# bbc/turingcodec

Measured on AMD Instinct MI355X. Metric: encoded fps (havoc hot path, primitive-batch throughput: one picture's primitive calls per frame as whole-frame batches;, higher is better.
Workload: dtype u8; 1 GPU; 1920x1080 8-bit 4:2:0 random-access QP32 speed=medium B-frame, MEASURED call mix of the reference encoder on this clip generator (profiles/r04_reference_call_mi; calls_per_frame=3944815, launches_per_frame=49, pictures_in_flight=2, parallelism=single GPU

## Files before the change

### turingcodec_amd/csrc/kernels_tu_fused.hip

```cpp
#include "common.h"

#include <cstdlib>
#include "transform_basis.h"
#include "launch.h"
#include "rdoq_work.h"

namespace havoc_gpu {

template <int S, int N>
__device__ __forceinline__ void load_sample_row(const char *p, uint32_t (&row)[N / 2])
{
    if (S == 1)
    {
        uint32_t b[N / 4];
        if (N == 4) b[0] = ld4(p);
        else if (N == 8)
        {
            const u32x2 v = ld8(p);
            b[0] = v.x; b[1] = v.y;
        }
        else
        {
#pragma unroll
            for (int q = 0; q < N / 16; ++q)
            {
                const u32x4 v = ld16(p + 16 * q);
                b[4 * q] = v.x; b[4 * q + 1] = v.y; b[4 * q + 2] = v.z; b[4 * q + 3] = v.w;
            }
        }
#pragma unroll
        for (int q = 0; q < N / 4; ++q)
        {
            row[2 * q] = __builtin_amdgcn_perm(0u, b[q], 0x0c010c00u);
            row[2 * q + 1] = __builtin_amdgcn_perm(0u, b[q], 0x0c030c02u);
        }
    }
    else
    {
        if (N == 4)
        {
            const u32x2 v = ld8(p);
            row[0] = v.x; row[1] = v.y;
        }
        else
        {
#pragma unroll
            for (int q = 0; q < N / 8; ++q)
            {
                const u32x4 v = ld16(p + 16 * q);
                row[4 * q] = v.x; row[4 * q + 1] = v.y; row[4 * q + 2] = v.z; row[4 * q + 3] = v.w;
            }
        }
    }
}

template <int S, int LOG2, int TR, bool SCAN = false>
__global__ __launch_bounds__(64) void k_tu_forward(int16_t *__restrict__ coeffs, const char *__restrict__ src, long stride_src,
                                                   const char *__restrict__ pred, long stride_pred, const int32_t *__restrict__ jobs, int njobs,
                                                   int bitDepth, const RdoqJob *__restrict__ rjobs = nullptr, int16_t *__restrict__ levels = nullptr,
                                                   RdoqWork *__restrict__ work = nullptr)
{
    constexpr int N = 1 << LOG2, TPW = 64 / N, LS = N + 2;
    __shared__ int16_t lds[TPW][N * LS];
    const int t = threadIdx.x / N, r = threadIdx.x % N;
    const int job = xcd_block(blockIdx.x, gridDim.x) * TPW + t;
    const bool live = job < njobs;
    const int32_t *j = jobs + (long)(live ? job : 0) * 4;
    const int shift1 = LOG2 - 1 + bitDepth - 8, shift2 = LOG2 + 6;

    uint32_t row[N / 2], prow[N / 2];
    load_sample_row<S, N>(src + ((long)j[1] + (long)r * stride_src) * S, row);
    load_sample_row<S, N>(pred + ((long)j[2] + (long)r * stride_pred) * S, prow);
#pragma unroll
    for (int p = 0; p < N / 2; ++p) row[p] = pk_sub(row[p], prow[p]);
    int o[N];
    basis_times_row<N, TR, false, true>(row, 1 << (shift1 - 1), o);
#pragma unroll
    for (int k = 0; k < N; ++k) lds[t][k * LS + r] = (int16_t)(o[k] >> shift1);
    __syncthreads();
#pragma unroll
    for (int p = 0; p < N / 2; ++p) row[p] = *reinterpret_cast<const uint32_t *>(&lds[t][r * LS + 2 * p]);
    basis_times_row<N, TR, false>(row, 1 << (shift2 - 1), o);
    if (SCAN)
    {
        constexpr int GW = N / 4;
        const RdoqJob rj = rjobs[live ? job : 0];
        uint32_t thr[3];
        rdoqThresholds(rj.quant_scale, rj.quant_shift, thr);
        uint32_t lo = 0, hi = 0;
        uint64_t mask[3] = {0, 0, 0};
#pragma unroll
        for (int gy = 0; gy < GW; ++gy)
        {
            uint32_t big = 0;
#pragma unroll
            for (int k = 4 * gy; k < 4 * gy + 4; ++k)
            {
                const int c = (int16_t)(o[k] >> shift2);
                big = max(big, (uint32_t)abs(c));
                const uint32_t sq = (uint32_t)(c * c);
                lo += sq & 0xffffu;
                hi += sq >> 16;
            }
            big = max(big, (uint32_t)__shfl_xor((int)big, 1, kWave));
            big = max(big, (uint32_t)__shfl_xor((int)big, 2, kWave));
#pragma unroll
            for (int m = 0; m < 3; ++m)
            {
                const uint64_t b = __ballot(live && (r & 3) == 0 && big >= thr[m]) >> (t * N);
                uint32_t f = 0;
#pragma unroll
                for (int gx = 0; gx < GW; ++gx) f |= (uint32_t)((b >> (4 * gx)) & 1) << gx;
                mask[m] |= (uint64_t)f << (gy * GW);
            }
        }
        const int slo = group_sum<N>((int)lo), shi = group_sum<N>((int)hi);
        if (live)
        {
            int16_t *z = levels + rj.dst_off + r * N;
#pragma unroll
            for (int q = 0; q < N / 4; ++q) st8(z + 4 * q, u32x2{0, 0});
            if (r == 0)
            {
                RdoqInfo *info = reinterpret_cast<RdoqInfo *>(reinterpret_cast<char *>(work) + rdoqInfoOffset());
                RdoqInfo v;
                v.mask = mask[0];
                v.mask2 = mask[1];
                v.mask3 = mask[2];
                v.sumSq = ((int64_t)shi << 16) + slo;
                info[job] = v;
            }
        }
    }
    if (!live) return;
    int16_t *c = coeffs + j[0] + r;
#pragma unroll
    for (int k = 0; k < N; ++k) c[k * N] = (int16_t)(o[k] >> shift2);
}

template <int S, int LOG2, int TR>
__global__ __launch_bounds__(64) void k_tu_reconstruct(char *rec, long stride_rec, const char *pred, long stride_pred, const char *__restrict__ src,
                                                       long stride_src, const int16_t *__restrict__ levels, const int32_t *__restrict__ jobs,
                                                       int njobs, int bitDepth, int scale, int shift, uint32_t *__restrict__ ssd)
{
    typedef typename Sample<S>::T T;
    constexpr int N = 1 << LOG2, TPW = 64 / N, LS = N + 2;
    __shared__ int16_t lds[TPW][N * LS];
    const int t = threadIdx.x / N, r = threadIdx.x % N;
    const int job = xcd_block(blockIdx.x, gridDim.x) * TPW + t;
    const bool live = job < njobs;
    const int32_t *j = jobs + (long)(live ? job : 0) * 4;
    const int shift2 = 20 - bitDepth;
    const int dqadd = 1 << (shift - 1);

    const int16_t *c = levels + j[0] + r;
    uint32_t col[N / 2];
#pragma unroll
    for (int p = 0; p < N / 2; ++p)
    {
        const int lo = clip3(-32768, 32767, ((int)c[(2 * p) * N] * scale + dqadd) >> shift);
        const int hi = clip3(-32768, 32767, ((int)c[(2 * p + 1) * N] * scale + dqadd) >> shift);
        col[p] = ((uint32_t)lo & 0xffffu) | ((uint32_t)hi << 16);
    }
    int o[N];
    basis_times_row<N, TR, true>(col, 1 << 6, o);
#pragma unroll
    for (int k = 0; k < N; ++k) lds[t][k * LS + r] = (int16_t)clip3(-32768, 32767, o[k] >> 7);
    __syncthreads();
#pragma unroll
    for (int p = 0; p < N / 2; ++p) col[p] = *reinterpret_cast<const uint32_t *>(&lds[t][r * LS + 2 * p]);
    basis_times_row<N, TR, true>(col, 1 << (shift2 - 1), o);

    const int maxv = (1 << bitDepth) - 1;
    uint32_t prow[N / 2], srow[N / 2];
    load_sample_row<S, N>(pred + ((long)j[2] + (long)r * stride_pred) * S, prow);
    load_sample_row<S, N>(src + ((long)j[1] + (long)r * stride_src) * S, srow);
    uint32_t acc = 0;
    int v[N];
#pragma unroll
    for (int k = 0; k < N; ++k)
    {
        const int res = clip3(-32768, 32767, o[k] >> shift2);
        const int pk = (k & 1) ? (int)(prow[k >> 1] >> 16) : (int)(prow[k >> 1] & 0xffff);
        const int sk = (k & 1) ? (int)(srow[k >> 1] >> 16) : (int)(srow[k >> 1] & 0xffff);
        v[k] = clip3(0, maxv, pk + res);
        const int d = sk - v[k];
        acc += (uint32_t)(d * d);
    }
    if (live)
    {
        T *q = reinterpret_cast<T *>(rec) + j[3] + (long)r * stride_rec;
        if (S == 1)
        {
#pragma unroll
            for (int k = 0; k < N; k += 4) st4(q + k, (uint32_t)v[k] | ((uint32_t)v[k + 1] << 8) | ((uint32_t)v[k + 2] << 16) | ((uint32_t)v[k + 3] << 24));
        }
        else
        {
#pragma unroll
            for (int k = 0; k < N; k += 2) st4(q + k, (uint32_t)v[k] | ((uint32_t)v[k + 1] << 16));
        }
    }
    uint32_t tot = (uint32_t)group_sum<N>((int)acc);
    if (S == 2) tot >>= 4;
    if (live && r == 0) ssd[job] = tot;
}

template <int S, int LOG2>
__global__ __launch_bounds__(64) void k_intra_measure(int16_t *__restrict__ coeffs, int16_t *__restrict__ coeffsDct, int32_t *__restrict__ satd, char *__restrict__ rec0,
                                                      uint32_t *__restrict__ ssd0, const char *__restrict__ src, long stride_src, const char *__restrict__ pred,
                                                      long stride_pred, const int32_t *__restrict__ jobs, int njobs, int bitDepth, int withSatd)
{
    typedef typename Sample<S>::T T;
    constexpr int N = 1 << LOG2, TPW = 64 / N, LS = N + 2, TS = N >= 8 ? 8 : 4, TX = N / TS, TILES = TX * TX;
    __shared__ int16_t lds[TPW][N * LS];
    const int t = threadIdx.x / N, r = threadIdx.x % N;
    const int job = blockIdx.x * TPW + t;
    const bool live = job < njobs;
    const int32_t *j = jobs + (long)(live ? job : 0) * 4;
    const int shift1 = LOG2 - 1 + bitDepth - 8, shift2 = LOG2 + 6;

    uint32_t row[N / 2], prow[N / 2];
    load_sample_row<S, N>(src + ((long)j[1] + (long)r * stride_src) * S, row);
    load_sample_row<S, N>(pred + ((long)j[2] + (long)r * stride_pred) * S, prow);
    if (live)
    {
        const int maxv = (1 << bitDepth) - 1;
        T *q = reinterpret_cast<T *>(rec0) + j[3] + (long)r * N;
#pragma unroll
        for (int p = 0; p < N / 2; ++p)
        {
            q[2 * p] = (T)clip3(0, maxv, (int)(prow[p] & 0xffff));
            q[2 * p + 1] = (T)clip3(0, maxv, (int)(prow[p] >> 16));
        }
    }
#pragma unroll
    for (int p = 0; p < N / 2; ++p) row[p] = pk_sub(row[p], prow[p]);
    {
        uint32_t acc = 0;
#pragma unroll
        for (int p = 0; p < N / 2; ++p)
        {
            const int lo = (int16_t)(row[p] & 0xffff), hi = (int16_t)(row[p] >> 16);
            acc += (uint32_t)(lo * lo) + (uint32_t)(hi * hi);
        }
        uint32_t tot = (uint32_t)group_sum<N>((int)acc);
        if (S == 2) tot >>= 4;
        if (live && r == 0) ssd0[job] = tot;
    }
    if (withSatd)
    {
#pragma unroll
        for (int tx = 0; tx < TX; ++tx)
        {
            int c;
            if (S == 1)
            {
                uint32_t p[TS / 2];
#pragma unroll
                for (int k = 0; k < TS / 2; ++k) p[k] = row[tx * (TS / 2) + k];
                c = satd_rows_pk<TS>(p, r & (TS - 1));
            }
            else
            {
                int d[TS];
#pragma unroll
                for (int k = 0; k < TS / 2; ++k)
                {
                    d[2 * k] = (int16_t)(row[tx * (TS / 2) + k] & 0xffff);
                    d[2 * k + 1] = (int16_t)(row[tx * (TS / 2) + k] >> 16);
                }
                c = satd_rows<S, TS>(d, r & (TS - 1));
            }
            if (live && (r & (TS - 1)) == 0) satd[(long)job * TILES + (r / TS) * TX + tx] = c;
        }
    }
    uint32_t keep[N / 2];
#pragma unroll
    for (int p = 0; p < N / 2; ++p) keep[p] = row[p];
    int o[N];
    constexpr int TR = LOG2 == 2 ? 1 : 0;
    basis_times_row<N, TR, false, true>(row, 1 << (shift1 - 1), o);
#pragma unroll
    for (int k = 0; k < N; ++k) lds[t][k * LS + r] = (int16_t)(o[k] >> shift1);
    __syncthreads();
#pragma unroll
    for (int p = 0; p < N / 2; ++p) row[p] = *reinterpret_cast<const uint32_t *>(&lds[t][r * LS + 2 * p]);
    basis_times_row<N, TR, false>(row, 1 << (shift2 - 1), o);
    if (live)
    {
        int16_t *c = coeffs + j[0] + r;
#pragma unroll
        for (int k = 0; k < N; ++k) c[k * N] = (int16_t)(o[k] >> shift2);
    }
    if (LOG2 == 2)
    {
        __syncthreads();
        basis_times_row<N, 0, false, true>(keep, 1 << (shift1 - 1), o);
#pragma unroll
        for (int k = 0; k < N; ++k) lds[t][k * LS + r] = (int16_t)(o[k] >> shift1);
        __syncthreads();
#pragma unroll
        for (int p = 0; p < N / 2; ++p) row[p] = *reinterpret_cast<const uint32_t *>(&lds[t][r * LS + 2 * p]);
        basis_times_row<N, 0, false>(row, 1 << (shift2 - 1), o);
        if (live)
        {
            int16_t *c = coeffsDct + j[0] + r;
#pragma unroll
            for (int k = 0; k < N; ++k) c[k * N] = (int16_t)(o[k] >> shift2);
        }
    }
}

hipError_t launch_intra_measure(hipStream_t st, int S, int bd, int log2, int16_t *coeffs, int16_t *coeffsDct, int32_t *satd, void *rec0, uint32_t *ssd0, const void *src,
                                long ss, const void *pred, long sp, const havoc_mi355x_tu_fused_job *jobs, int n, int withSatd)
{
    if (n <= 0) return hipSuccess;
    if (log2 < 2 || log2 > 5) return hipErrorInvalidValue;
    const int tpw = 64 >> log2;
    const dim3 g((n + tpw - 1) / tpw), b(64);
    char *r0 = (char *)rec0;
    const char *s8 = (const char *)src, *p8 = (const char *)pred;
    const int32_t *j = (const int32_t *)jobs;
#define MEASURE_GO(SS, LL) hipLaunchKernelGGL((k_intra_measure<SS, LL>), g, b, 0, st, coeffs, coeffsDct, satd, r0, ssd0, s8, ss, p8, sp, j, n, bd, withSatd)
    if (S == 1) { if (log2 == 2) MEASURE_GO(1, 2); else if (log2 == 3) MEASURE_GO(1, 3); else if (log2 == 4) MEASURE_GO(1, 4); else MEASURE_GO(1, 5); }
    else { if (log2 == 2) MEASURE_GO(2, 2); else if (log2 == 3) MEASURE_GO(2, 3); else if (log2 == 4) MEASURE_GO(2, 4); else MEASURE_GO(2, 5); }
#undef MEASURE_GO
    return hipGetLastError();
}


typedef int i32x16v __attribute__((ext_vector_type(16)));
typedef int i32x4v __attribute__((ext_vector_type(4)));

struct Dct32I8 { int8_t m[32][32]; int32_t rowsum128[32]; };
constexpr Dct32I8 make_dct32_i8()
{
    Dct32I8 t{};
    for (int k = 0; k < 32; ++k)
    {
        int sum = 0;
        for (int c = 0; c < 32; ++c)
        {
            t.m[k][c] = (int8_t)basis(32, 0, k, c);
            sum += basis(32, 0, k, c);
        }
        t.rowsum128[k] = 128 * sum;
    }
    return t;
}
static __constant__ Dct32I8 c_dct32_i8 = make_dct32_i8();

__device__ __forceinline__ void mfma_dct32(const i32x4v a, const uint32_t (&v)[8], int add, int half, int (&out)[16])
{
    i32x4v bh, bl;
#pragma unroll
    for (int q = 0; q < 4; ++q)
    {
        bh[q] = (int)__builtin_amdgcn_perm(v[2 * q + 1], v[2 * q], 0x07050301u);
        bl[q] = (int)(__builtin_amdgcn_perm(v[2 * q + 1], v[2 * q], 0x06040200u) ^ 0x80808080u);
    }
    i32x16v ch, cl;
#pragma unroll
    for (int reg = 0; reg < 16; ++reg)
    {
        ch[reg] = 0;
        cl[reg] = add + c_dct32_i8.rowsum128[(reg & 3) + 8 * (reg >> 2) + 4 * half];
    }
    ch = __builtin_amdgcn_mfma_i32_32x32x32_i8(a, bh, ch, 0, 0, 0);
    cl = __builtin_amdgcn_mfma_i32_32x32x32_i8(a, bl, cl, 0, 0, 0);
#pragma unroll
    for (int reg = 0; reg < 16; ++reg) out[reg] = (int)(((uint32_t)ch[reg] << 8) + (uint32_t)cl[reg]);
}

template <bool SCAN>
__global__ __launch_bounds__(64) void k_tu_forward_mfma32(int16_t *__restrict__ coeffs, const char *__restrict__ src, long stride_src, const char *__restrict__ pred,
                                                          long stride_pred, const int32_t *__restrict__ jobs, int njobs, const RdoqJob *__restrict__ rjobs = nullptr,
                                                          int16_t *__restrict__ levels = nullptr, RdoqWork *__restrict__ work = nullptr)
{
    constexpr int LS = 40;
    __shared__ __attribute__((aligned(16))) int16_t lds[32 * LS];
    const int job = xcd_block(blockIdx.x, gridDim.x);
    if (job >= njobs) return;
    const int32_t *j = jobs + (long)job * 4;
    const int lane = threadIdx.x, y = lane & 31, half = lane >> 5;
    const i32x4v a = *reinterpret_cast<const i32x4v *>(&c_dct32_i8.m[y][16 * half]);
    uint32_t r[8];
    {
        const u32x4 s4 = ld16(src + (long)j[1] + (long)y * stride_src + 16 * half), p4 = ld16(pred + (long)j[2] + (long)y * stride_pred + 16 * half);
        const uint32_t sw[4] = {s4.x, s4.y, s4.z, s4.w}, pw[4] = {p4.x, p4.y, p4.z, p4.w};
#pragma unroll
        for (int q = 0; q < 4; ++q)
        {
            r[2 * q] = pk_sub(__builtin_amdgcn_perm(0u, sw[q], 0x0c010c00u), __builtin_amdgcn_perm(0u, pw[q], 0x0c010c00u));
            r[2 * q + 1] = pk_sub(__builtin_amdgcn_perm(0u, sw[q], 0x0c030c02u), __builtin_amdgcn_perm(0u, pw[q], 0x0c030c02u));
        }
    }
    int t[16];
    mfma_dct32(a, r, 8, half, t);
#pragma unroll
    for (int reg = 0; reg < 16; ++reg) lds[((reg & 3) + 8 * (reg >> 2) + 4 * half) * LS + y] = (int16_t)(t[reg] >> 4);
    __syncthreads();
    uint32_t v[8];
    {
        const u32x4 q0 = *reinterpret_cast<const u32x4 *>(&lds[y * LS + 16 * half]), q1 = *reinterpret_cast<const u32x4 *>(&lds[y * LS + 16 * half + 8]);
        v[0] = q0.x; v[1] = q0.y; v[2] = q0.z; v[3] = q0.w; v[4] = q1.x; v[5] = q1.y; v[6] = q1.z; v[7] = q1.w;
    }
    int o[16];
    mfma_dct32(a, v, 1024, half, o);
    int16_t *c = coeffs + j[0] + y;
#pragma unroll
    for (int reg = 0; reg < 16; ++reg) c[((reg & 3) + 8 * (reg >> 2) + 4 * half) * 32] = (int16_t)(o[reg] >> 11);
    if (SCAN)
    {
        const RdoqJob rj = rjobs[job];
        uint32_t thr[3];
        rdoqThresholds(rj.quant_scale, rj.quant_shift, thr);
        uint32_t lo = 0, hi = 0;
        uint64_t mask[3] = {0, 0, 0};
#pragma unroll
        for (int q = 0; q < 4; ++q)
        {
            uint32_t big = 0;
#pragma unroll
            for (int k = 0; k < 4; ++k)
            {
                const int cf = (int16_t)(o[4 * q + k] >> 11);
                big = max(big, (uint32_t)abs(cf));
                const uint32_t sq = (uint32_t)(cf * cf);
                lo += sq & 0xffffu;
                hi += sq >> 16;
            }
            big = max(big, (uint32_t)__shfl_xor((int)big, 1, kWave));
            big = max(big, (uint32_t)__shfl_xor((int)big, 2, kWave));
#pragma unroll
            for (int m = 0; m < 3; ++m)
            {
                const uint64_t b = __ballot((y & 3) == 0 && big >= thr[m]);
                uint32_t f0 = 0, f1 = 0;
#pragma unroll
                for (int gx = 0; gx < 8; ++gx)
                {
                    f0 |= (uint32_t)((b >> (4 * gx)) & 1) << gx;
                    f1 |= (uint32_t)((b >> (32 + 4 * gx)) & 1) << gx;
                }
                mask[m] |= (uint64_t)f0 << (16 * q) | (uint64_t)f1 << (16 * q + 8);
            }
        }
        const int slo = wave_sum((int)lo), shi = wave_sum((int)hi);
        int16_t *z = levels + rj.dst_off + lane * 16;
        st8(z, u32x2{0, 0}); st8(z + 4, u32x2{0, 0}); st8(z + 8, u32x2{0, 0}); st8(z + 12, u32x2{0, 0});
        if (lane == 0)
        {
            RdoqInfo *info = reinterpret_cast<RdoqInfo *>(reinterpret_cast<char *>(work) + rdoqInfoOffset());
            RdoqInfo w;
            w.mask = mask[0];
            w.mask2 = mask[1];
            w.mask3 = mask[2];
            w.sumSq = ((int64_t)shi << 16) + slo;
            info[job] = w;
        }
    }
}

static bool mfmaForward()
{
    static const bool on = !(getenv("HAVOC_TU_MFMA") && atoi(getenv("HAVOC_TU_MFMA")) == 0);
    return on;
}

template <int S, int LOG2, int TR>
static void go_fwd(hipStream_t st, int16_t *co, const char *src, long ss, const char *pred, long sp, const int32_t *j, int n, int bd)
{
    constexpr int TPW = 64 >> LOG2;
    hipLaunchKernelGGL((k_tu_forward<S, LOG2, TR>), dim3((n + TPW - 1) / TPW), dim3(64), 0, st, co, src, ss, pred, sp, j, n, bd);
}

template <int S>
static hipError_t launch_fwd_s(hipStream_t st, int bd, int log2, int tr, int16_t *co, const char *src, long ss, const char *pred, long sp,
                               const int32_t *j, int n)
{
    if (tr)
    {
        if (log2 != 2) return hipErrorInvalidValue;
        go_fwd<S, 2, 1>(st, co, src, ss, pred, sp, j, n, bd);
    }
    else
        switch (log2)
        {
        case 2: go_fwd<S, 2, 0>(st, co, src, ss, pred, sp, j, n, bd); break;
        case 3: go_fwd<S, 3, 0>(st, co, src, ss, pred, sp, j, n, bd); break;
        case 4: go_fwd<S, 4, 0>(st, co, src, ss, pred, sp, j, n, bd); break;
        case 5:
            if (S == 1 && bd == 8 && mfmaForward()) hipLaunchKernelGGL((k_tu_forward_mfma32<false>), dim3(n), dim3(64), 0, st, co, src, ss, pred, sp, j, n);
            else go_fwd<S, 5, 0>(st, co, src, ss, pred, sp, j, n, bd);
            break;
        default: return hipErrorInvalidValue;
        }
    return hipGetLastError();
}

hipError_t launch_tu_forward_scan(hipStream_t st, int S, int bd, int log2, int16_t *coeffs, const void *src, long ss, const void *pred, long sp,
                                  const havoc_mi355x_tu_fused_job *jobs, int n, const RdoqJob *rj, int16_t *levels, void *workspace)
{
    if (n <= 0) return hipSuccess;
    if (log2 != 4 && log2 != 5) return hipErrorInvalidValue;
    const char *s8 = (const char *)src, *p8 = (const char *)pred;
    const int32_t *j = (const int32_t *)jobs;
    RdoqWork *w = (RdoqWork *)workspace;
    const int tpw = 64 >> log2;
    const dim3 g((n + tpw - 1) / tpw), b(64);
    if (S == 1 && log2 == 4) hipLaunchKernelGGL((k_tu_forward<1, 4, 0, true>), g, b, 0, st, coeffs, s8, ss, p8, sp, j, n, bd, rj, levels, w);
    else if (S == 1 && bd == 8 && mfmaForward()) hipLaunchKernelGGL((k_tu_forward_mfma32<true>), dim3(n), b, 0, st, coeffs, s8, ss, p8, sp, j, n, rj, levels, w);
    else if (S == 1) hipLaunchKernelGGL((k_tu_forward<1, 5, 0, true>), g, b, 0, st, coeffs, s8, ss, p8, sp, j, n, bd, rj, levels, w);
    else if (log2 == 4) hipLaunchKernelGGL((k_tu_forward<2, 4, 0, true>), g, b, 0, st, coeffs, s8, ss, p8, sp, j, n, bd, rj, levels, w);
    else hipLaunchKernelGGL((k_tu_forward<2, 5, 0, true>), g, b, 0, st, coeffs, s8, ss, p8, sp, j, n, bd, rj, levels, w);
    return hipGetLastError();
}

hipError_t launch_tu_forward(hipStream_t st, int S, int bd, int log2, int tr, int16_t *coeffs, const void *src, long ss, const void *pred, long sp,
                             const havoc_mi355x_tu_fused_job *jobs, int n)
{
    if (n <= 0) return hipSuccess;
    return S == 1 ? launch_fwd_s<1>(st, bd, log2, tr, coeffs, (const char *)src, ss, (const char *)pred, sp, (const int32_t *)jobs, n)
                  : launch_fwd_s<2>(st, bd, log2, tr, coeffs, (const char *)src, ss, (const char *)pred, sp, (const int32_t *)jobs, n);
}

template <int S, int LOG2, int TR>
static void go_rec(hipStream_t st, char *rec, long sr, const char *pred, long sp, const char *src, long ss, const int16_t *lv, const int32_t *j, int n,
                   int bd, int scale, int shift, uint32_t *ssd)
{
    constexpr int TPW = 64 >> LOG2;
    hipLaunchKernelGGL((k_tu_reconstruct<S, LOG2, TR>), dim3((n + TPW - 1) / TPW), dim3(64), 0, st, rec, sr, pred, sp, src, ss, lv, j, n, bd, scale,
                       shift, ssd);
}

template <int S>
static hipError_t launch_rec_s(hipStream_t st, int bd, int log2, int tr, int scale, int shift, char *rec, long sr, const char *pred, long sp,
                               const char *src, long ss, const int16_t *lv, const int32_t *j, int n, uint32_t *ssd)
{
    if (tr)
    {
        if (log2 != 2) return hipErrorInvalidValue;
        go_rec<S, 2, 1>(st, rec, sr, pred, sp, src, ss, lv, j, n, bd, scale, shift, ssd);
    }
    else
        switch (log2)
        {
        case 2: go_rec<S, 2, 0>(st, rec, sr, pred, sp, src, ss, lv, j, n, bd, scale, shift, ssd); break;
        case 3: go_rec<S, 3, 0>(st, rec, sr, pred, sp, src, ss, lv, j, n, bd, scale, shift, ssd); break;
        case 4: go_rec<S, 4, 0>(st, rec, sr, pred, sp, src, ss, lv, j, n, bd, scale, shift, ssd); break;
        case 5: go_rec<S, 5, 0>(st, rec, sr, pred, sp, src, ss, lv, j, n, bd, scale, shift, ssd); break;
        default: return hipErrorInvalidValue;
        }
    return hipGetLastError();
}

hipError_t launch_tu_reconstruct(hipStream_t st, int S, int bd, int log2, int tr, int scale, int shift, void *rec, long sr, const void *pred, long sp,
                                 const void *src, long ss, const int16_t *levels, const havoc_mi355x_tu_fused_job *jobs, int n, uint32_t *ssd)
{
    if (n <= 0) return hipSuccess;
    return S == 1 ? launch_rec_s<1>(st, bd, log2, tr, scale, shift, (char *)rec, sr, (const char *)pred, sp, (const char *)src, ss, levels,
                                    (const int32_t *)jobs, n, ssd)
                  : launch_rec_s<2>(st, bd, log2, tr, scale, shift, (char *)rec, sr, (const char *)pred, sp, (const char *)src, ss, levels,
                                    (const int32_t *)jobs, n, ssd);
}

}
```

### turingcodec_amd/csrc/transform_basis.h

```cpp
#pragma once

#include "common.h"

namespace havoc_gpu {

constexpr int kMag[33] = {64, 90, 90, 90, 89, 88, 87, 85, 83, 82, 80, 78, 75, 73, 70, 67, 64,
                          61, 57, 54, 50, 46, 43, 38, 36, 31, 25, 22, 18, 13, 9,  4,  0};
constexpr int kDst7[4][4] = {{29, 55, 74, 84}, {74, 74, 0, -74}, {84, -29, -74, 55}, {55, -84, 74, -29}};

constexpr int basis(int n, int tr, int k, int c)
{
    if (tr) return kDst7[k][c];
    const int kk = k * (32 / n);
    if (kk == 0) return 64;
    const int j = (kk * (2 * c + 1)) & 127;
    return j <= 32 ? kMag[j] : (j <= 64 ? -kMag[64 - j] : (j <= 96 ? -kMag[j - 64] : kMag[128 - j]));
}

template <int N> struct PackedBasis { uint32_t v[N][N / 2]; };

template <int N, int TR, bool INV>
constexpr PackedBasis<N> make_basis()
{
    PackedBasis<N> m{};
    for (int k = 0; k < N; ++k)
        for (int p = 0; p < N / 2; ++p)
        {
            const int lo = INV ? basis(N, TR, 2 * p, k) : basis(N, TR, k, 2 * p);
            const int hi = INV ? basis(N, TR, 2 * p + 1, k) : basis(N, TR, k, 2 * p + 1);
            m.v[k][p] = ((uint32_t)lo & 0xffffu) | ((uint32_t)hi << 16);
        }
    return m;
}

static __constant__ PackedBasis<4> c_fwd_dst4 = make_basis<4, 1, false>();
static __constant__ PackedBasis<4> c_fwd_dct4 = make_basis<4, 0, false>();
static __constant__ PackedBasis<8> c_fwd_dct8 = make_basis<8, 0, false>();
static __constant__ PackedBasis<16> c_fwd_dct16 = make_basis<16, 0, false>();
static __constant__ PackedBasis<32> c_fwd_dct32 = make_basis<32, 0, false>();
static __constant__ PackedBasis<4> c_inv_dst4 = make_basis<4, 1, true>();
static __constant__ PackedBasis<4> c_inv_dct4 = make_basis<4, 0, true>();
static __constant__ PackedBasis<8> c_inv_dct8 = make_basis<8, 0, true>();
static __constant__ PackedBasis<16> c_inv_dct16 = make_basis<16, 0, true>();
static __constant__ PackedBasis<32> c_inv_dct32 = make_basis<32, 0, true>();

template <int N, int TR, bool INV> __device__ __forceinline__ const PackedBasis<N> &basis_table();
template <> __device__ __forceinline__ const PackedBasis<4> &basis_table<4, 1, false>() { return c_fwd_dst4; }
template <> __device__ __forceinline__ const PackedBasis<4> &basis_table<4, 0, false>() { return c_fwd_dct4; }
template <> __device__ __forceinline__ const PackedBasis<8> &basis_table<8, 0, false>() { return c_fwd_dct8; }
template <> __device__ __forceinline__ const PackedBasis<16> &basis_table<16, 0, false>() { return c_fwd_dct16; }
template <> __device__ __forceinline__ const PackedBasis<32> &basis_table<32, 0, false>() { return c_fwd_dct32; }
template <> __device__ __forceinline__ const PackedBasis<4> &basis_table<4, 1, true>() { return c_inv_dst4; }
template <> __device__ __forceinline__ const PackedBasis<4> &basis_table<4, 0, true>() { return c_inv_dct4; }
template <> __device__ __forceinline__ const PackedBasis<8> &basis_table<8, 0, true>() { return c_inv_dct8; }
template <> __device__ __forceinline__ const PackedBasis<16> &basis_table<16, 0, true>() { return c_inv_dct16; }
template <> __device__ __forceinline__ const PackedBasis<32> &basis_table<32, 0, true>() { return c_inv_dct32; }

__device__ __forceinline__ int dot2(uint32_t a, uint32_t b, int c)
{
    return __builtin_amdgcn_sdot2(__builtin_bit_cast(s16x2, a), __builtin_bit_cast(s16x2, b), c, false);
}


template <int N> struct PackedBasisEO { uint32_t ve[N / 2][N / 4], vo[N / 2][N / 4]; };

template <int N>
constexpr PackedBasisEO<N> make_basis_eo()
{
    PackedBasisEO<N> m{};
    for (int i = 0; i < N / 2; ++i)
        for (int q = 0; q < N / 4; ++q)
        {
            m.ve[i][q] = ((uint32_t)basis(N, 0, 4 * q, i) & 0xffffu) | ((uint32_t)basis(N, 0, 4 * q + 2, i) << 16);
            m.vo[i][q] = ((uint32_t)basis(N, 0, 4 * q + 1, i) & 0xffffu) | ((uint32_t)basis(N, 0, 4 * q + 3, i) << 16);
        }
    return m;
}
static __constant__ PackedBasisEO<16> c_eo_dct16 = make_basis_eo<16>();
static __constant__ PackedBasisEO<32> c_eo_dct32 = make_basis_eo<32>();
template <int N> __device__ __forceinline__ const PackedBasisEO<N> &basis_eo();
template <> __device__ __forceinline__ const PackedBasisEO<16> &basis_eo<16>() { return c_eo_dct16; }
template <> __device__ __forceinline__ const PackedBasisEO<32> &basis_eo<32>() { return c_eo_dct32; }

template <int N, int TR, bool INV, bool FOLD = false>
__device__ __forceinline__ void basis_times_row(const uint32_t (&row)[N / 2], int add, int (&out)[N])
{
    if constexpr (INV && TR == 0 && N >= 16)
    {
        const PackedBasisEO<N> &m = basis_eo<N>();
        uint32_t ce[N / 4], co[N / 4];
#pragma unroll
        for (int q = 0; q < N / 4; ++q)
        {
            ce[q] = __builtin_amdgcn_perm(row[2 * q + 1], row[2 * q], 0x05040100u);
            co[q] = __builtin_amdgcn_perm(row[2 * q + 1], row[2 * q], 0x07060302u);
        }
#pragma unroll
        for (int i = 0; i < N / 2; ++i)
        {
            int e = add, o = 0;
#pragma unroll
            for (int q = 0; q < N / 4; ++q)
            {
                e = dot2(ce[q], m.ve[i][q], e);
                o = dot2(co[q], m.vo[i][q], o);
            }
            out[i] = e + o;
            out[N - 1 - i] = e - o;
        }
    }
    else if constexpr (!INV && TR == 0 && N >= 16 && FOLD)
    {
        const PackedBasis<N> &m = basis_table<N, TR, INV>();
        uint32_t ev[N / 4], od[N / 4];
#pragma unroll
        for (int p = 0; p < N / 4; ++p)
        {
            const uint32_t b = row[N / 2 - 1 - p];
            const uint32_t bs = __builtin_amdgcn_alignbit(b, b, 16);
            ev[p] = pk_add(row[p], bs);
            od[p] = pk_sub(row[p], bs);
        }
#pragma unroll
        for (int k = 0; k < N; ++k)
        {
            int a = add;
#pragma unroll
            for (int p = 0; p < N / 4; ++p) a = dot2((k & 1) ? od[p] : ev[p], m.v[k][p], a);
            out[k] = a;
        }
    }
    else
    {
        const PackedBasis<N> &m = basis_table<N, TR, INV>();
#pragma unroll
        for (int k = 0; k < N; ++k)
        {
            int a = add;
#pragma unroll
            for (int p = 0; p < N / 2; ++p) a = dot2(row[p], m.v[k][p], a);
            out[k] = a;
        }
    }
}

template <int N>
__device__ __forceinline__ void load_row16(const int16_t *p, uint32_t (&row)[N / 2])
{
    if (N == 4)
    {
        const u32x2 v = ld8(p);
        row[0] = v.x; row[1] = v.y;
    }
    else
    {
#pragma unroll
        for (int q = 0; q < N / 8; ++q)
        {
            const u32x4 v = ld16(p + 8 * q);
            row[4 * q] = v.x; row[4 * q + 1] = v.y; row[4 * q + 2] = v.z; row[4 * q + 3] = v.w;
        }
    }
}

}
```

Before: 1610 frames/s.

## Skip zero coefficient regions in TU reconstruct via wavefront-uniform extent

The reconstruct kernel now finds, across the wavefront, the highest nonzero row and column band of the quantized levels using ballots. It dispatches truncated inverse-transform passes that only multiply over the first 4/8/16 inputs, and skips both passes when every level is zero. It also packs the add/clip/SSD math into 16-bit pairs with saturating ops and dot2, issues the pred/src loads early for small sizes, and reduces the SSD with DPP into the last lane. The cost is more template instantiations and branches, which means higher code size and register pressure. The savings depend on how sparse the levels are per wavefront.

```diff
diff --git a/profiles/level_extent.py b/profiles/level_extent.py
--- /dev/null
+++ b/profiles/level_extent.py
@@ -0,0 +1,72 @@
+#!/usr/bin/env python3
+import argparse
+import os
+import sys
+from collections import Counter
+
+import numpy as np
+
+ROOT = os.path.dirname(os.path.dirname(os.path.abspath(__file__)))
+sys.path.insert(0, ROOT)
+sys.path.insert(0, os.path.join(ROOT, "tests"))
+from turingcodec_amd.workload import FrameWorkload, quant_params, dequant_params
+from reflibs import Oracle
+
+
+def cls(k, n):
+    return 0 if k == 0 else next(c for c in (4, 8, 16, 32) if k <= c or c >= n)
+
+
+def levels_of(o, wl, g, log2, tr, i):
+    n, st = g["n"], wl.stride
+    so, po = int(g["src"][i, 0]), int(g["src"][i, 1])
+    sblk = np.stack([wl.luma[so + r * st: so + r * st + n] for r in range(n)]).astype(np.int32)
+    pblk = np.stack([wl.luma[po + r * st: po + r * st + n] for r in range(n)]).astype(np.int32)
+    res = np.ascontiguousarray((sblk - pblk).astype(np.int16).ravel())
+    coef = np.zeros(n * n, np.int16)
+    o.transform(coef, 0, res, 0, n, log2, tr, wl.bit_depth)
+    qs, qsh, _ = quant_params(wl.qp, log2, wl.bit_depth, False)
+    inv, _ = dequant_params(wl.qp, log2, wl.bit_depth)
+    lv, _ = o.rdoq(coef, log2, 0, int(g["scan_idx"][i]), int(g["is_intra"][i]), 1, qs, qsh, inv, wl.bit_depth, wl.rdoq_lambda, wl.rdoq_states[g["ctx_index"][i]])
+    return np.asarray(lv).reshape(n, n)
+
+
+def extents(wl, waves, seed=1):
+    o = Oracle()
+    rng = np.random.default_rng(seed)
+    out = {}
+    for (log2, tr), g in sorted(wl.tu.items()):
+        n = g["n"]
+        tpw = 64 // n
+        nw = len(g["jobs"]) // tpw
+        per_block, per_wave = Counter(), Counter()
+        for w in rng.choice(nw, min(waves, nw), replace=False):
+            kr = kc = 0
+            for i in range(w * tpw, (w + 1) * tpw):
+                nz = levels_of(o, wl, g, log2, tr, i) != 0
+                rows, cols = np.flatnonzero(nz.any(1)), np.flatnonzero(nz.any(0))
+                r, c = (cls(rows[-1] + 1, n), cls(cols[-1] + 1, n)) if len(rows) else (0, 0)
+                per_block[(r, c)] += 1
+                kr, kc = max(kr, r), max(kc, c)
+            per_wave[(kr, kc)] += 1
+        out[(log2, tr)] = (tpw, per_block, per_wave)
+    return out
+
+
+def show(c):
+    tot = sum(c.values())
+    return "  ".join(f"{'zero' if k == (0, 0) else '%dx%d' % k} {100.0 * v / tot:.1f}%" for k, v in sorted(c.items()))
+
+
+if __name__ == "__main__":
+    ap = argparse.ArgumentParser()
+    ap.add_argument("--qp", type=int, default=32)
+    ap.add_argument("--waves", type=int, default=300)
+    a = ap.parse_args()
+    wl = FrameWorkload(1920, 1080, 8, 11, qp=a.qp)
+    print(f"FrameWorkload(1920, 1080, 8, 11, qp={a.qp}): extent of the levels, rows x columns rounded up to 0 / 4 / 8 / 16 / N; {a.waves} wavefronts per size")
+    for (log2, tr), (tpw, blocks, waves) in extents(wl, a.waves).items():
+        n = 1 << log2
+        print(f"{n}x{n} {'DST' if tr else 'DCT'}  ({tpw} blocks per wavefront, {sum(blocks.values())} blocks sampled)")
+        print(f"    per block      {show(blocks)}")
+        print(f"    per wavefront  {show(waves)}")
diff --git a/profiles/r07/tu_reconstruct_sparse_counts.py b/profiles/r07/tu_reconstruct_sparse_counts.py
--- /dev/null
+++ b/profiles/r07/tu_reconstruct_sparse_counts.py
@@ -0,0 +1,42 @@
+#!/usr/bin/env python3
+import csv
+import glob
+import os
+import re
+import sys
+
+
+def rows(d, pattern):
+    for f in sorted(glob.glob(os.path.join(d, "**", pattern), recursive=True)):
+        with open(f) as fh:
+            yield from csv.DictReader(fh)
+
+
+def inst(name):
+    m = re.search(r"k_tu_reconstruct<([^>]*)>", name)
+    return m.group(1).replace(" ", "") if m else name
+
+
+def main(pmc, trace, steps):
+    launches = []
+    for r in rows(pmc, "*counter_collection.csv"):
+        if r.get("Counter_Name") == "SQ_INSTS_VALU" and "k_tu_reconstruct" in r["Kernel_Name"]:
+            launches.append((int(r.get("Dispatch_Id", len(launches))), inst(r["Kernel_Name"]), int(r.get("Grid_Size", 0)) // max(int(r.get("Workgroup_Size", 64)), 1),
+                             float(r["Counter_Value"])))
+    launches.sort()
+    per = len(launches) // steps if steps else len(launches)
+    print(f"{len(launches)} k_tu_reconstruct launches in {steps} steps ({per} per step); S, LOG2, TR | workgroups (one wavefront each) | SQ_INSTS_VALU | per wavefront")
+    for i, (_, k, wg, v) in enumerate(launches):
+        if steps and i % per == 0:
+            print(f"  step {i // per}")
+        print(f"    <{k}>  {wg:7d}  {v:12.0f}  {v / wg if wg else 0:8.1f}")
+    if launches:
+        print(f"  sum per step: {sum(v for *_, v in launches) / max(steps, 1):.0f}")
+    for r in rows(trace, "*kernel_stats.csv"):
+        if "k_tu_reconstruct" in r.get("Name", ""):
+            print(f"  trace <{inst(r['Name'])}>  calls {r.get('Calls')}  total {float(r.get('TotalDurationNs', 0)) / 1e3:.1f} us  average {float(r.get('AverageNs', 0)) / 1e3:.2f} us"
+                  f"  min {float(r.get('MinNs', 0)) / 1e3:.2f}  max {float(r.get('MaxNs', 0)) / 1e3:.2f}")
+
+
+if __name__ == "__main__":
+    main(sys.argv[1], sys.argv[2], int(sys.argv[3]) if len(sys.argv) > 3 else 2)
diff --git a/turingcodec_amd/csrc/kernels_tu_fused.hip b/turingcodec_amd/csrc/kernels_tu_fused.hip
--- a/turingcodec_amd/csrc/kernels_tu_fused.hip
+++ b/turingcodec_amd/csrc/kernels_tu_fused.hip
@@ -8,50 +8,47 @@
 namespace havoc_gpu {
 
 template <int S, int N>
-__device__ __forceinline__ void load_sample_row(const char *p, uint32_t (&row)[N / 2])
-{
-    if (S == 1)
-    {
-        uint32_t b[N / 4];
-        if (N == 4) b[0] = ld4(p);
-        else if (N == 8)
-        {
-            const u32x2 v = ld8(p);
-            b[0] = v.x; b[1] = v.y;
-        }
-        else
-        {
-#pragma unroll
-            for (int q = 0; q < N / 16; ++q)
-            {
-                const u32x4 v = ld16(p + 16 * q);
-                b[4 * q] = v.x; b[4 * q + 1] = v.y; b[4 * q + 2] = v.z; b[4 * q + 3] = v.w;
-            }
-        }
-#pragma unroll
-        for (int q = 0; q < N / 4; ++q)
+__device__ __forceinline__ void load_sample_bytes(const char *p, uint32_t (&b)[N * S / 4])
+{
+    constexpr int BYTES = N * S;
+    if (BYTES == 4) b[0] = ld4(p);
+    else if (BYTES == 8)
+    {
+        const u32x2 v = ld8(p);
+        b[0] = v.x; b[1] = v.y;
+    }
+    else
+    {
+#pragma unroll
+        for (int q = 0; q < BYTES / 16; ++q)
+        {
+            const u32x4 v = ld16(p + 16 * q);
+            b[4 * q] = v.x; b[4 * q + 1] = v.y; b[4 * q + 2] = v.z; b[4 * q + 3] = v.w;
+        }
+    }
+}
+
+template <int S, int N>
+__device__ __forceinline__ void unpack_sample_row(const uint32_t (&b)[N * S / 4], uint32_t (&row)[N / 2])
+{
+#pragma unroll
+    for (int q = 0; q < N * S / 4; ++q)
+    {
+        if (S == 1)
         {
             row[2 * q] = __builtin_amdgcn_perm(0u, b[q], 0x0c010c00u);
             row[2 * q + 1] = __builtin_amdgcn_perm(0u, b[q], 0x0c030c02u);
         }
-    }
-    else
-    {
-        if (N == 4)
-        {
-            const u32x2 v = ld8(p);
-            row[0] = v.x; row[1] = v.y;
-        }
-        else
-        {
-#pragma unroll
-            for (int q = 0; q < N / 8; ++q)
-            {
-                const u32x4 v = ld16(p + 16 * q);
-                row[4 * q] = v.x; row[4 * q + 1] = v.y; row[4 * q + 2] = v.z; row[4 * q + 3] = v.w;
-            }
-        }
-    }
+        else row[q] = b[q];
+    }
+}
+
+template <int S, int N>
+__device__ __forceinline__ void load_sample_row(const char *p, uint32_t (&row)[N / 2])
+{
+    uint32_t b[N * S / 4];
+    load_sample_bytes<S, N>(p, b);
+    unpack_sample_row<S, N>(b, row);
 }
 
 template <int S, int LOG2, int TR, bool SCAN = false>
@@ -138,6 +135,49 @@
     for (int k = 0; k < N; ++k) c[k * N] = (int16_t)(o[k] >> shift2);
 }
 
+template <int G>
+__device__ __forceinline__ int group_sum_last(int v)
+{
+    v += __builtin_amdgcn_update_dpp(0, v, 0x111, 0xf, 0xf, true);
+    v += __builtin_amdgcn_update_dpp(0, v, 0x112, 0xf, 0xf, true);
+    if (G >= 8) v += __builtin_amdgcn_update_dpp(0, v, 0x114, 0xf, 0xe, true);
+    if (G >= 16) v += __builtin_amdgcn_update_dpp(0, v, 0x118, 0xf, 0xc, true);
+    if (G >= 32) v += __builtin_amdgcn_update_dpp(0, v, 0x142, 0xa, 0xf, true);
+    return v;
+}
+
+__device__ __forceinline__ uint32_t pack_sat(int lo, int hi) { return __builtin_bit_cast(uint32_t, __builtin_amdgcn_cvt_pk_i16(lo, hi)); }
+
+template <int N, int TR, int KR>
+__device__ __forceinline__ void rec_pass1(const int (&lv)[N], int scale, int dqadd, int shift, int16_t *ldsCol)
+{
+    constexpr int LS = N + 2;
+    uint32_t col[N / 2];
+#pragma unroll
+    for (int p = 0; p < KR / 2; ++p) col[p] = pack_sat((lv[2 * p] * scale + dqadd) >> shift, (lv[2 * p + 1] * scale + dqadd) >> shift);
+    int o[N];
+    basis_times_row<N, TR, true, false, KR>(col, 1 << 6, o);
+#pragma unroll
+    for (int k = 0; k < N; k += 2)
+    {
+        const s16x2 pr = __builtin_amdgcn_cvt_pk_i16(o[k] >> 7, o[k + 1] >> 7);
+        ldsCol[k * LS] = pr.x;
+        ldsCol[(k + 1) * LS] = pr.y;
+    }
+}
+
+template <int N, int TR, int KC>
+__device__ __forceinline__ void rec_pass2(const int16_t *ldsRow, int shift2, uint32_t (&res)[N / 2])
+{
+    uint32_t row[N / 2];
+#pragma unroll
+    for (int p = 0; p < KC / 2; ++p) row[p] = *reinterpret_cast<const uint32_t *>(&ldsRow[2 * p]);
+    int o[N];
+    basis_times_row<N, TR, true, false, KC>(row, 1 << (shift2 - 1), o);
+#pragma unroll
+    for (int p = 0; p < N / 2; ++p) res[p] = pack_sat(o[2 * p] >> shift2, o[2 * p + 1] >> shift2);
+}
+
 template <int S, int LOG2, int TR>
 __global__ __launch_bounds__(64) void k_tu_reconstruct(char *rec, long stride_rec, const char *pred, long stride_pred, const char *__restrict__ src,
                                                        long stride_src, const int16_t *__restrict__ levels, const int32_t *__restrict__ jobs,
@@ -145,65 +185,109 @@
 {
     typedef typename Sample<S>::T T;
     constexpr int N = 1 << LOG2, TPW = 64 / N, LS = N + 2;
+    constexpr int K4 = 4, K8 = N < 8 ? N : 8, K16 = N < 16 ? N : 16;
     __shared__ int16_t lds[TPW][N * LS];
     const int t = threadIdx.x / N, r = threadIdx.x % N;
     const int job = xcd_block(blockIdx.x, gridDim.x) * TPW + t;
     const bool live = job < njobs;
     const int32_t *j = jobs + (long)(live ? job : 0) * 4;
+    const int coef_off = j[0], src_off = j[1], pred_off = j[2], rec_off = j[3];
     const int shift2 = 20 - bitDepth;
     const int dqadd = 1 << (shift - 1);
 
-    const int16_t *c = levels + j[0] + r;
-    uint32_t col[N / 2];
+    const int16_t *c = levels + coef_off + r;
+    int lv[N];
+#pragma unroll
+    for (int k = 0; k < N; ++k) lv[k] = c[k * N];
+    constexpr bool EARLY = N < 32;
+    const char *prow_at = pred + ((long)pred_off + (long)r * stride_pred) * S, *srow_at = src + ((long)src_off + (long)r * stride_src) * S;
+    uint32_t pbytes[N * S / 4], sbytes[N * S / 4];
+    if (EARLY)
+    {
+        load_sample_bytes<S, N>(prow_at, pbytes);
+        load_sample_bytes<S, N>(srow_at, sbytes);
+    }
+
+    int from16 = 0, from8 = 0, from4 = 0, any = 0;
+#pragma unroll
+    for (int k = 0; k < N; ++k)
+    {
+        if (k >= 16) from16 |= lv[k];
+        else if (k >= 8) from8 |= lv[k];
+        else if (k >= 4) from4 |= lv[k];
+        else any |= lv[k];
+    }
+    from8 |= from16;
+    from4 |= from8;
+    any |= from4;
+    const uint64_t lives = __builtin_amdgcn_ballot_w64(live);
+    uint64_t cols = __builtin_amdgcn_ballot_w64(any != 0) & lives;
+    const bool rows4 = (__builtin_amdgcn_ballot_w64(from4 != 0) & lives) != 0, rows8 = (__builtin_amdgcn_ballot_w64(from8 != 0) & lives) != 0,
+               rows16 = (__builtin_amdgcn_ballot_w64(from16 != 0) & lives) != 0;
+    const int kr = __builtin_amdgcn_readfirstlane(cols == 0 ? 0 : rows16 ? 32 : rows8 ? 16 : rows4 ? 8 : 4);
+#pragma unroll
+    for (int w = 32; w >= N; w >>= 1) cols |= cols >> w;
+    const uint32_t field = (uint32_t)cols & (uint32_t)((1ull << N) - 1);
+    const int kc = __builtin_amdgcn_readfirstlane(field == 0 ? 0 : (field >> 16) ? 32 : (field >> 8) ? 16 : (field >> 4) ? 8 : 4);
+
+    uint32_t res[N / 2];
+    if (kr == 0)
+    {
+#pragma unroll
+        for (int p = 0; p < N / 2; ++p) res[p] = 0;
+    }
+    else
+    {
+        int16_t *ldsCol = &lds[t][r];
+        if (kr <= K4) rec_pass1<N, TR, K4>(lv, scale, dqadd, shift, ldsCol);
+        else if (kr <= K8) rec_pass1<N, TR, K8>(lv, scale, dqadd, shift, ldsCol);
+        else if (kr <= K16) rec_pass1<N, TR, K16>(lv, scale, dqadd, shift, ldsCol);
+        else rec_pass1<N, TR, N>(lv, scale, dqadd, shift, ldsCol);
+        __syncthreads();
+        const int16_t *ldsRow = &lds[t][r * LS];
+        if (kc <= K4) rec_pass2<N, TR, K4>(ldsRow, shift2, res);
+        else if (kc <= K8) rec_pass2<N, TR, K8>(ldsRow, shift2, res);
+        else if (kc <= K16) rec_pass2<N, TR, K16>(ldsRow, shift2, res);
+        else rec_pass2<N, TR, N>(ldsRow, shift2, res);
+    }
+
+    const uint32_t maxv = (uint32_t)((1 << bitDepth) - 1) * 0x10001u;
+    if (!EARLY)
+    {
+        load_sample_bytes<S, N>(prow_at, pbytes);
+        load_sample_bytes<S, N>(srow_at, sbytes);
+    }
+    uint32_t prow[N / 2], srow[N / 2];
+    unpack_sample_row<S, N>(pbytes, prow);
+    unpack_sample_row<S, N>(sbytes, srow);
+    int acc = 0;
+    uint32_t v[N / 2];
 #pragma unroll
     for (int p = 0; p < N / 2; ++p)
     {
-        const int lo = clip3(-32768, 32767, ((int)c[(2 * p) * N] * scale + dqadd) >> shift);
-        const int hi = clip3(-32768, 32767, ((int)c[(2 * p + 1) * N] * scale + dqadd) >> shift);
-        col[p] = ((uint32_t)lo & 0xffffu) | ((uint32_t)hi << 16);
-    }
-    int o[N];
-    basis_times_row<N, TR, true>(col, 1 << 6, o);
-#pragma unroll
-    for (int k = 0; k < N; ++k) lds[t][k * LS + r] = (int16_t)clip3(-32768, 32767, o[k] >> 7);
-    __syncthreads();
-#pragma unroll
-    for (int p = 0; p < N / 2; ++p) col[p] = *reinterpret_cast<const uint32_t *>(&lds[t][r * LS + 2 * p]);
-    basis_times_row<N, TR, true>(col, 1 << (shift2 - 1), o);
-
-    const int maxv = (1 << bitDepth) - 1;
-    uint32_t prow[N / 2], srow[N / 2];
-    load_sample_row<S, N>(pred + ((long)j[2] + (long)r * stride_pred) * S, prow);
-    load_sample_row<S, N>(src + ((long)j[1] + (long)r * stride_src) * S, srow);
-    uint32_t acc = 0;
-    int v[N];
-#pragma unroll
-    for (int k = 0; k < N; ++k)
-    {
-        const int res = clip3(-32768, 32767, o[k] >> shift2);
-        const int pk = (k & 1) ? (int)(prow[k >> 1] >> 16) : (int)(prow[k >> 1] & 0xffff);
-        const int sk = (k & 1) ? (int)(srow[k >> 1] >> 16) : (int)(srow[k >> 1] & 0xffff);
-        v[k] = clip3(0, maxv, pk + res);
-        const int d = sk - v[k];
-        acc += (uint32_t)(d * d);
+        s16x2 x = __builtin_elementwise_add_sat(__builtin_bit_cast(s16x2, prow[p]), __builtin_bit_cast(s16x2, res[p]));
+        x = __builtin_elementwise_min(__builtin_elementwise_max(x, (s16x2){0, 0}), __builtin_bit_cast(s16x2, maxv));
+        v[p] = __builtin_bit_cast(uint32_t, x);
+        const uint32_t d = pk_sub(srow[p], v[p]);
+        acc = dot2(d, d, acc);
     }
     if (live)
     {
-        T *q = reinterpret_cast<T *>(rec) + j[3] + (long)r * stride_rec;
+        T *q = reinterpret_cast<T *>(rec) + rec_off + (long)r * stride_rec;
         if (S == 1)
         {
 #pragma unroll
-            for (int k = 0; k < N; k += 4) st4(q + k, (uint32_t)v[k] | ((uint32_t)v[k + 1] << 8) | ((uint32_t)v[k + 2] << 16) | ((uint32_t)v[k + 3] << 24));
+            for (int k = 0; k < N; k += 4) st4(q + k, __builtin_amdgcn_perm(v[k / 2 + 1], v[k / 2], 0x06040200u));
         }
         else
         {
 #pragma unroll
-            for (int k = 0; k < N; k += 2) st4(q + k, (uint32_t)v[k] | ((uint32_t)v[k + 1] << 16));
-        }
-    }
-    uint32_t tot = (uint32_t)group_sum<N>((int)acc);
+            for (int k = 0; k < N; k += 2) st4(q + k, v[k / 2]);
+        }
+    }
+    uint32_t tot = (uint32_t)group_sum_last<N>(acc);
     if (S == 2) tot >>= 4;
-    if (live && r == 0) ssd[job] = tot;
+    if (live && r == N - 1) ssd[job] = tot;
 }
 
 template <int S, int LOG2>
diff --git a/turingcodec_amd/csrc/transform_basis.h b/turingcodec_amd/csrc/transform_basis.h
--- a/turingcodec_amd/csrc/transform_basis.h
+++ b/turingcodec_amd/csrc/transform_basis.h
@@ -82,15 +82,16 @@
 template <> __device__ __forceinline__ const PackedBasisEO<16> &basis_eo<16>() { return c_eo_dct16; }
 template <> __device__ __forceinline__ const PackedBasisEO<32> &basis_eo<32>() { return c_eo_dct32; }
 
-template <int N, int TR, bool INV, bool FOLD = false>
+template <int N, int TR, bool INV, bool FOLD = false, int K = N>
 __device__ __forceinline__ void basis_times_row(const uint32_t (&row)[N / 2], int add, int (&out)[N])
 {
+    static_assert(K >= 4 && K <= N && K % 4 == 0 && (K == N || !FOLD), "K: a multiple of 4 up to N, the full length with FOLD");
     if constexpr (INV && TR == 0 && N >= 16)
     {
         const PackedBasisEO<N> &m = basis_eo<N>();
-        uint32_t ce[N / 4], co[N / 4];
+        uint32_t ce[K / 4], co[K / 4];
 #pragma unroll
-        for (int q = 0; q < N / 4; ++q)
+        for (int q = 0; q < K / 4; ++q)
         {
             ce[q] = __builtin_amdgcn_perm(row[2 * q + 1], row[2 * q], 0x05040100u);
             co[q] = __builtin_amdgcn_perm(row[2 * q + 1], row[2 * q], 0x07060302u);
@@ -100,7 +101,7 @@
         {
             int e = add, o = 0;
 #pragma unroll
-            for (int q = 0; q < N / 4; ++q)
+            for (int q = 0; q < K / 4; ++q)
             {
                 e = dot2(ce[q], m.ve[i][q], e);
                 o = dot2(co[q], m.vo[i][q], o);
@@ -138,7 +139,7 @@
         {
             int a = add;
 #pragma unroll
-            for (int p = 0; p < N / 2; ++p) a = dot2(row[p], m.v[k][p], a);
+            for (int p = 0; p < K / 2; ++p) a = dot2(row[p], m.v[k][p], a);
             out[k] = a;
         }
     }
```

Result: slower. 1585 frames/s (-1.5%).
